# alisher-turubayev/dl-normalizing-flows

Measured on AMD Instinct MI355X. Metric: images/sec + bits/dim, RealNVP 64x64x3 training, higher is better.
Workload: dtype bf16; 1 GPU; config 1: RealNVP 64x64x3, res-blocks 4, base-dim 32, per-GPU batch 64, train step fwd+bwd+Adam; global_batch=64, image_size=64, res_blocks=4, base_dim=32, n_scales=5, parallelism=dp1, graph=True, side_stream=False

## Files before the change

### dl-normalizing-flows_amd/csrc/conv.hip

```cpp
#include <math.h>
#include <stdlib.h>

#include "common.h"
#include "conv_common.h"

#ifndef RNVP_SHARD_PX
#define RNVP_SHARD_PX 8192
#endif
extern "C" int rnvp_stat_shards(long long M) {
    long long s = M / RNVP_SHARD_PX;
    int r = 1;
    while (r < 32 && r * 2 <= s) r *= 2;
    return r;
}

namespace {

int conv_args_status(const rnvp_conv_args* a) {
    if (!a || !a->x || !a->w || !a->y) return RNVP_E_INVALID;
    if (a->variant < 0 || (a->variant > RNVP_VARIANT_DEEP && a->variant < RNVP_VARIANT_DEEP0) ||
        a->variant >= RNVP_VARIANT_DEEP0 + RNVP_DEEP_CFGS)
        return RNVP_E_INVALID;
    if (a->w_frag && !al16(a->w_frag)) return RNVP_E_INVALID;
    if (a->dtype != RNVP_F32 && a->dtype != RNVP_BF16) return RNVP_E_INVALID;
    if (a->ks != 1 && a->ks != 3) return RNVP_E_UNSUPPORTED;
    if (a->B < 0 || a->H <= 0 || a->W <= 0 || a->n <= 0 || a->cin <= 0) return RNVP_E_INVALID;
    if ((a->cs_in & 7) || (a->cs_out & 7) || a->cs_in < a->cin || a->cs_out < a->n) return RNVP_E_INVALID;
    if ((a->kp & 63) || a->kp < a->ks * a->ks * a->cs_in) return RNVP_E_INVALID;
    if (!al16(a->x) || !al16(a->w)) return RNVP_E_INVALID;
    if (a->epi_relu_bn_bwd && !a->epi_x) return RNVP_E_INVALID;
    auto tab_bad = [](const rnvp_bn_src& s) { return s.tab && (!s.sums || !al16(s.tab)); };
    if ((a->pro_bn_relu && tab_bad(a->pro)) || (a->epi_relu_bn_bwd && tab_bad(a->epi)) || (a->bp && tab_bad(a->bp_bn)))
        return RNVP_E_INVALID;
    if ((long long)a->B * a->H * a->W >= (1ll << 31)) return RNVP_E_UNSUPPORTED;
    if (a->bp) {
        if (!a->bp_x || !al16(a->bp_x) || (a->bp_out && !al16(a->bp_out))) return RNVP_E_INVALID;
        if (a->bp_bn.sums && (!a->bp_sums || a->bp_shards < 1 || a->bp_bn.count <= 0)) return RNVP_E_INVALID;
        if (!a->bp_bn.sums && (!a->bp_bn.mean || !a->bp_bn.var)) return RNVP_E_INVALID;
        if (a->pro_bn_relu) return RNVP_E_INVALID;
    }
    return RNVP_OK;
}

int bp_cfg_of(const rnvp_conv_args* a) {
    if (a->variant >= RNVP_VARIANT_DEEP0) {
        const int cfg = a->variant - RNVP_VARIANT_DEEP0;
        return (cfg == 0 || cfg == 4) ? cfg : -1;
    }
    if (a->variant != 0 && a->variant != RNVP_VARIANT_DEEP) return -1;
    const int cfg = rnvp_deep_auto_cfg(a);
    const long long M = (long long)a->B * a->H * a->W;
    if (cfg == 4 || (cfg == 0 && (a->ks == 3 || M <= 4096))) return cfg;
    return -1;
}

int dispatch_conv(const rnvp_conv_args* a, hipStream_t s, bool dry, int* fam) {
    auto ran = [&](int f, int r) {
        if (fam && r == RNVP_OK) *fam = f;
        return r;
    };
    if (a->variant >= RNVP_VARIANT_DEEP0)
        return ran(RNVP_FAMILY_DEEP, rnvp_deep_launch(a, s, a->variant - RNVP_VARIANT_DEEP0, dry));
    if (a->variant == 0 || a->variant == RNVP_VARIANT_DEEP) {
        const int cfg = rnvp_deep_auto_cfg(a);
        if (cfg >= 0) {
            const int r = rnvp_deep_launch(a, s, cfg, dry);
            if (r != RNVP_E_UNSUPPORTED) return ran(RNVP_FAMILY_DEEP, r);
        }
    }
    const bool tuned = a->variant != 1;
    if (tuned && a->dtype == RNVP_BF16 && a->ks == 1) {
        const int r = rnvp_conv_s1_launch(a, s, dry);
        if (r != RNVP_E_UNSUPPORTED) return ran(RNVP_FAMILY_S1, r);
    }
    if (tuned && rnvp_conv_band_ok(a)) {
        const int r = rnvp_conv_band2_launch(a, s, dry);
        if (r != RNVP_E_UNSUPPORTED) return ran(RNVP_FAMILY_BAND, r);
        if (dry) return ran(RNVP_FAMILY_OTHER, RNVP_OK);
        return rnvp_conv_band1_launch(a, s);
    }
    if (dry) return ran(RNVP_FAMILY_OTHER, RNVP_OK);
    {
        const int r = rnvp_conv_stream_launch(a, s);
        if (r != RNVP_E_UNSUPPORTED) return r;
    }
    if (tuned) {
        const int r = rnvp_conv_halo_launch(a, s);
        if (r != RNVP_E_UNSUPPORTED) return r;
    }
    return rnvp_conv_tiled_launch(a, s);
}

int route_conv(const rnvp_conv_args* a, hipStream_t s, bool dry, int* fam = nullptr) {
    if (a->bp) {
        const int cfg = bp_cfg_of(a);
        int r, f = RNVP_FAMILY_DEEP;
        if (cfg >= 0) {
            r = rnvp_deep_launch(a, s, cfg, dry);
        } else {
            if (a->variant != 0) return RNVP_E_UNSUPPORTED;
            f = RNVP_FAMILY_S1;
            r = rnvp_conv_s1_launch(a, s, dry);
            if (r == RNVP_E_UNSUPPORTED) {
                f = RNVP_FAMILY_BAND;
                r = rnvp_conv_band2_launch(a, s, dry);
            }
        }
        if (fam && r == RNVP_OK) *fam = f;
        return r;
    }
    return dispatch_conv(a, s, dry, fam);
}

}

extern "C" int rnvp_conv2d(const rnvp_conv_args* a, void* stream) {
    const int st = conv_args_status(a);
    if (st != RNVP_OK || a->B == 0) return st;
    return route_conv(a, (hipStream_t)stream, false);
}

extern "C" int rnvp_conv2d_family(const rnvp_conv_args* a) {
    const int st = conv_args_status(a);
    if (st != RNVP_OK) return st;
    int fam = RNVP_FAMILY_OTHER;
    const int r = route_conv(a, nullptr, true, &fam);
    return r == RNVP_OK ? fam : r;
}

extern "C" int rnvp_conv2d_check(const rnvp_conv_args* a) {
    const int st = conv_args_status(a);
    if (st != RNVP_OK || a->B == 0) return st;
    return route_conv(a, nullptr, true);
}
```

### dl-normalizing-flows_amd/csrc/conv_common.h

```cpp
#pragma once
#include <math.h>

#include "common.h"

namespace {

template <typename T> struct Mf;
template <> struct Mf<bf16_t> {
    static constexpr int CH = 8;
    __device__ static __forceinline__ void step(const u32x4& a, const u32x4& b, floatx4& c) {
        c = __builtin_amdgcn_mfma_f32_16x16x32_bf16(__builtin_bit_cast(bf16x8, a), __builtin_bit_cast(bf16x8, b), c, 0, 0, 0);
    }
};
template <> struct Mf<float> {
    static constexpr int CH = 4;
    __device__ static __forceinline__ void step(const u32x4& a, const u32x4& b, floatx4& c) {
        c = __builtin_amdgcn_mfma_f32_16x16x4f32(__uint_as_float(a.x), __uint_as_float(b.x), c, 0, 0, 0);
        c = __builtin_amdgcn_mfma_f32_16x16x4f32(__uint_as_float(a.y), __uint_as_float(b.y), c, 0, 0, 0);
        c = __builtin_amdgcn_mfma_f32_16x16x4f32(__uint_as_float(a.z), __uint_as_float(b.z), c, 0, 0, 0);
        c = __builtin_amdgcn_mfma_f32_16x16x4f32(__uint_as_float(a.w), __uint_as_float(b.w), c, 0, 0, 0);
    }
};

__device__ __forceinline__ int sw8(int row, int c) { return row * 8 + (c ^ ((row >> 1) & 7)); }
// ... 314 lines not shown
        float g[CH], x[CH], d[CH];
        unpack(vg, g, T());
        unpack(vx, x, T());
#pragma unroll
        for (int j = 0; j < CH; ++j) {
            const float* pp = p + 5 * (c0 + j);
            const float xh = (x[j] - pp[3]) * pp[4];
            d[j] = pp[0] * (g[j] - pp[1] - xh * pp[2]);
        }
        if (R) {
            float r[CH];
            unpack(vr, r, T());
#pragma unroll
            for (int j = 0; j < CH; ++j) d[j] += r[j];
        }
        if (a.accumulate) {
            float r[CH];
            unpack(vd, r, T());
#pragma unroll
            for (int j = 0; j < CH; ++j) d[j] += r[j];
        }
        *(u32x4*)(DX + o) = pack(d, T());
    };
    if (q0 < nch) apply(q0 * CH, fg, fx, fr, fd);
    for (long long q = q0 + qs; q < nch; q += qs) {
        const long long o = q * CH;
        if (!fixed) c0 = (int)(q % cpr) * CH;
        const u32x4 vg = *(const u32x4*)(G + o), vx = *(const u32x4*)(X + o);
        const u32x4 vr = R ? *(const u32x4*)(R + o) : vg;
        const u32x4 vd = a.accumulate ? *(const u32x4*)(DX + o) : vg;
        apply(o, vg, vx, vr, vd);
    }
}

template <typename T>
__device__ __forceinline__ void bn_bwd_body(const rnvp_bn_bwd_args& a, double* dsm, int blk, int nblk) {
    if (a.bn.gamma) bn_bwd_run<T, true>(a, dsm, blk, nblk);
    else bn_bwd_run<T, false>(a, dsm, blk, nblk);
}

inline bool al16(const void* p) { return (((uintptr_t)p) & 15) == 0; }

}

int rnvp_conv_tiled_launch(const rnvp_conv_args* a, hipStream_t s);

int rnvp_conv_stream_launch(const rnvp_conv_args* a, hipStream_t s);

int rnvp_conv_halo_launch(const rnvp_conv_args* a, hipStream_t s);

bool rnvp_conv_band_ok(const rnvp_conv_args* a);
int rnvp_conv_band1_launch(const rnvp_conv_args* a, hipStream_t s);

constexpr int RNVP_DEEP_CFGS = 7;
int rnvp_deep_launch(const rnvp_conv_args* a, hipStream_t s, int cfg, bool dry = false);
int rnvp_deep_auto_cfg(const rnvp_conv_args* a);

int rnvp_wgrad_tap_launch(rnvp_wgrad_group* g, hipStream_t s);
int rnvp_wgrad_tap_prepare(rnvp_wgrad_group* g);
int rnvp_wgrad_tap_multi_plan(const rnvp_wgrad_group* groups, int n_groups, int cls, rnvp_wgrad_multi_conv* convs,
                              int conv_cap, int* xcd_start, int* tasks, int task_cap, rnvp_wgrad_multi* m);
int rnvp_wgrad_tap_multi_launch(const rnvp_wgrad_multi* m, hipStream_t s);

int rnvp_conv_s1_launch(const rnvp_conv_args* a, hipStream_t s, bool dry = false);

struct rnvp_group_kargs {
    rnvp_conv_args conv[RNVP_NET_GROUP_MAX];
    int shards[RNVP_NET_GROUP_MAX], tiles[RNVP_NET_GROUP_MAX], xa[RNVP_NET_GROUP_MAX], xb[RNVP_NET_GROUP_MAX];
    int n;
};
rnvp_group_kargs group_kargs(const rnvp_net_step* steps, int n);

using GroupKernel = void (*)(const rnvp_group_kargs);
template <typename T, int CFG> int rnvp_deep_cfg_launch(const rnvp_conv_args* a, hipStream_t s, bool dry);
template <typename T, int CFG> GroupKernel rnvp_deep_cfg_group(int nc, bool fm);
int rnvp_s1_fanout_prepare(rnvp_net_step* steps, int n, int* klass, int* grid, int* lds_bytes);
int rnvp_s1_fanout_launch(const rnvp_group_kargs& g, int klass, int grid, int lds_bytes, hipStream_t s);

int rnvp_conv_band2_launch(const rnvp_conv_args* a, hipStream_t s, bool dry = false);
```

### dl-normalizing-flows_amd/csrc/conv_deep.hip

```cpp
#include "conv_deep.h"

#ifdef RNVP_DEEP_STAMPS
#include "conv_deep_launch.h"
#endif

namespace {

template <typename T>
int launch_cfg(const rnvp_conv_args* a, hipStream_t s, int cfg, bool dry) {
    switch (cfg) {
        case 0: return rnvp_deep_cfg_launch<T, 0>(a, s, dry);
        case 1: return rnvp_deep_cfg_launch<T, 1>(a, s, dry);
        case 2: return rnvp_deep_cfg_launch<T, 2>(a, s, dry);
        case 3: return rnvp_deep_cfg_launch<T, 3>(a, s, dry);
        case 4: return rnvp_deep_cfg_launch<T, 4>(a, s, dry);
        case 5: return rnvp_deep_cfg_launch<T, 5>(a, s, dry);
        case 6: return rnvp_deep_cfg_launch<T, 6>(a, s, dry);
    }
    return RNVP_E_INVALID;
}

template <typename T>
GroupKernel group_kernel_t(int cfg, int nc, bool fm) {
    switch (cfg) {
        case 0: return rnvp_deep_cfg_group<T, 0>(nc, fm);
        case 1: return rnvp_deep_cfg_group<T, 1>(nc, fm);
        case 4: return rnvp_deep_cfg_group<T, 4>(nc, fm);
        case 5: return rnvp_deep_cfg_group<T, 5>(nc, fm);
    }
    return nullptr;
}

constexpr int GROUP_FM = 1 << 11;
GroupKernel group_kernel(int dtype, int klass) {
    const int cfg = klass & 15, nc = (klass >> 4) & 127;
    const bool fm = (klass & GROUP_FM) != 0;
    return dtype == RNVP_F32 ? group_kernel_t<float>(cfg, nc, fm) : group_kernel_t<bf16_t>(cfg, nc, fm);
}

struct GroupCfg { int bn, nw, wk; };
inline GroupCfg group_cfg_shape(int cfg) {
    switch (cfg) {
        case 0: return {32, 4, 4};
        case 1: return {64, 4, 4};
        case 4: return {32, 8, 8};
        default: return {64, 8, 8};
    }
}

}

extern "C" int rnvp_net_group_prepare(rnvp_net_step* steps, int n, int* klass, int* grid, int* lds_bytes) {
    if (!steps || n <= 0 || n > RNVP_NET_GROUP_MAX || !klass || !grid || !lds_bytes) return RNVP_E_INVALID;
    const rnvp_conv_args& a0 = steps[0].conv;
    const long long M = (long long)a0.B * a0.H * a0.W;
    for (int i = 0; i < n; ++i)
        if (steps[i].conv.bp) return RNVP_E_UNSUPPORTED;
    if (M > 16384) return rnvp_s1_fanout_prepare(steps, n, klass, grid, lds_bytes);
    if (M <= 0) return RNVP_E_UNSUPPORTED;
    if (a0.dtype != RNVP_F32 && a0.dtype != RNVP_BF16) return RNVP_E_INVALID;
    const int kc = a0.dtype == RNVP_F32 ? 16 : 32;
    int cfg = -1, nc = -1;
    long long tiles = 0;
    size_t lds = 0;
    for (int i = 0; i < n; ++i) {
        rnvp_net_step& st = steps[i];
        const rnvp_conv_args& a = st.conv;
        if (st.kind != RNVP_STEP_CONV || a.ks != 1) return RNVP_E_UNSUPPORTED;
        if (a.dtype != a0.dtype || a.B != a0.B || a.H != a0.H || a.W != a0.W) return RNVP_E_UNSUPPORTED;
        if (!a.x || !a.w || !a.y || a.n <= 0 || a.cin <= 0 || (a.cs_in & 7) || (a.cs_out & 7)) return RNVP_E_INVALID;
// ... 29 lines not shown
        st.cfg = c;
        st.nc = ncv;
        st.shards = rnvp_stat_shards(M);
        st.tiles = (int)(gm * gn);
        xcd_blocks(&a, (int)gm, (int)gn, g.bn, a0.dtype == RNVP_F32 ? 4 : 2, &st.xa, &st.xb);
        tiles += st.tiles;
    }
    if (tiles <= 0 || tiles >= (1ll << 31)) return RNVP_E_INVALID;
    bool fm = a0.dtype == RNVP_BF16 && nc <= 4;
    for (int i = 0; i < n; ++i) fm = fm && steps[i].conv.w_frag != nullptr && (((uintptr_t)steps[i].conv.w_frag) & 15) == 0;
    *klass = cfg | (nc << 4) | (fm ? GROUP_FM : 0);
    *grid = (int)tiles;
    *lds_bytes = (int)lds;
    return group_kernel(a0.dtype, *klass) ? RNVP_OK : RNVP_E_UNSUPPORTED;
}

rnvp_group_kargs group_kargs(const rnvp_net_step* steps, int n) {
    rnvp_group_kargs g = {};
    for (int i = 0; i < n; ++i) {
        g.conv[i] = steps[i].conv;
        g.shards[i] = steps[i].shards;
        g.tiles[i] = steps[i].tiles;
        g.xa[i] = steps[i].xa;
        g.xb[i] = steps[i].xb;
    }
    g.n = n;
    return g;
}

extern "C" int rnvp_net_group(const rnvp_net_step* steps, int n, int dtype, int klass, int grid, int lds_bytes,
                              void* stream) {
    if (!steps || n <= 0 || n > RNVP_NET_GROUP_MAX || grid <= 0 || lds_bytes < 0 || lds_bytes > 160 * 1024)
        return RNVP_E_INVALID;
    if (dtype != RNVP_F32 && dtype != RNVP_BF16) return RNVP_E_INVALID;
    const rnvp_group_kargs g = group_kargs(steps, n);
    if (klass & (1 << 12)) {
        if (dtype != RNVP_BF16 || n < 2) return RNVP_E_INVALID;
        return rnvp_s1_fanout_launch(g, klass, grid, lds_bytes, (hipStream_t)stream);
    }
    const GroupKernel k = group_kernel(dtype, klass);
    if (!k) return RNVP_E_INVALID;
    const int nw = group_cfg_shape(klass & 15).nw;
    hipLaunchKernelGGL(k, dim3(grid), dim3(64 * nw), lds_bytes, (hipStream_t)stream, g);
    RNVP_LAUNCH_CHECK();
    return RNVP_OK;
}

int rnvp_deep_auto_cfg(const rnvp_conv_args* a) {
    const long long M = (long long)a->B * a->H * a->W;
    if (M > 16384) return -1;
    const bool dgrad = a->epi_relu_bn_bwd || (!a->pro_bn_relu && !a->out_sums);
    const int kc = a->dtype == RNVP_F32 ? 16 : 32;
    if (M <= 1024) return a->cs_in % (8 * kc) == 0 ? 4 : 0;
    if (dgrad) return 0;
    if (a->ks == 3 && a->dtype == RNVP_BF16 && M > 4096 && a->cs_in == 128) return 6;
    return a->cs_in % (8 * kc) == 0 ? 5 : 1;
}

int rnvp_deep_launch(const rnvp_conv_args* a, hipStream_t s, int cfg, bool dry) {
    if (cfg < 0 || cfg >= RNVP_DEEP_CFGS) return RNVP_E_INVALID;
    return a->dtype == RNVP_F32 ? launch_cfg<float>(a, s, cfg, dry) : launch_cfg<bf16_t>(a, s, cfg, dry);
}
```

### dl-normalizing-flows_amd/csrc/conv_deep_launch.h

```cpp
#pragma once
#include "conv_deep.h"

namespace {

template <typename T, int BN, int KSZ, bool PRO, int NW, int WK, int DK, int NC, bool FM = false, int BM = DEEP_BM,
          bool BP = false>
__global__ __launch_bounds__(64 * NW) void k_conv_deep(rnvp_conv_args a, int shards, int xa, int xb) {
    extern __shared__ __attribute__((aligned(16))) char lds[];
    deep_tile<T, BN, KSZ, PRO, NW, WK, DK, NC, FM, BM, BP>(a, shards, xa, xb, blockIdx.x, gridDim.x, lds);
}

template <int BN, int NW, int WK, int BM>
constexpr bool bp_cfg() { return BN == 32 && WK == NW && BM == DEEP_BM; }

template <typename T, int BN, int NW, int WK, int DK, int NC, int KSZ, int BM = DEEP_BM>
int launch_deep_nc(const rnvp_conv_args* a, hipStream_t s, bool dry) {
    const long long M = (long long)a->B * a->H * a->W;
    const size_t shm = deep_lds_bytes<T, BN, NW, WK, BM>(a->cs_in, a->W, a->ks, a->bp != 0);
    if (shm > 160 * 1024) return RNVP_E_UNSUPPORTED;
    const long long gm = (M + BM - 1) / BM, gn = (a->n + BN - 1) / BN;
    const unsigned grid = (unsigned)(gm * gn);
    const int sh = rnvp_stat_shards(M);
    const dim3 blk(64 * NW);
    int xa, xb;
    xcd_blocks(a, (int)gm, (int)gn, BN, sizeof(T), &xa, &xb, BM);
    if (a->bp) {
        if constexpr (bp_cfg<BN, NW, WK, BM>()) {
            if (dry) return RNVP_OK;
            if constexpr (sizeof(T) == 2 && NC <= 4) {
                if (a->w_frag) {
                    k_conv_deep<T, BN, KSZ, false, NW, WK, DK, NC, true, BM, true><<<grid, blk, shm, s>>>(*a, sh, xa, xb);
                    RNVP_LAUNCH_CHECK();
                    return RNVP_OK;
                }
            }
            k_conv_deep<T, BN, KSZ, false, NW, WK, DK, NC, false, BM, true><<<grid, blk, shm, s>>>(*a, sh, xa, xb);
            RNVP_LAUNCH_CHECK();
            return RNVP_OK;
        } else {
            return RNVP_E_UNSUPPORTED;
        }
    }
    if (dry) return RNVP_OK;
    if constexpr (sizeof(T) == 2 && NC <= 4) {
        if (a->w_frag) {
            if (a->pro_bn_relu) k_conv_deep<T, BN, KSZ, true, NW, WK, DK, NC, true, BM><<<grid, blk, shm, s>>>(*a, sh, xa, xb);
            else k_conv_deep<T, BN, KSZ, false, NW, WK, DK, NC, true, BM><<<grid, blk, shm, s>>>(*a, sh, xa, xb);
            RNVP_LAUNCH_CHECK();
            return RNVP_OK;
        }
    }
    if (a->pro_bn_relu) k_conv_deep<T, BN, KSZ, true, NW, WK, DK, NC, false, BM><<<grid, blk, shm, s>>>(*a, sh, xa, xb);
    else k_conv_deep<T, BN, KSZ, false, NW, WK, DK, NC, false, BM><<<grid, blk, shm, s>>>(*a, sh, xa, xb);
    RNVP_LAUNCH_CHECK();
// ... 49 lines not shown
        return RNVP_E_UNSUPPORTED;
    }
}

template <typename T, int BN, int NW, int WK, int DK, int NC, bool FM = false>
__global__ __launch_bounds__(64 * NW) void k_net_group(const rnvp_group_kargs g) {
    extern __shared__ __attribute__((aligned(16))) char lds[];
    int b = blockIdx.x, c = 0;
    while (c + 1 < g.n && b >= g.tiles[c]) {
        b -= g.tiles[c];
        ++c;
    }
    if (g.conv[c].pro_bn_relu)
        deep_tile<T, BN, 1, true, NW, WK, DK, NC, FM>(g.conv[c], g.shards[c], g.xa[c], g.xb[c], b, g.tiles[c], lds);
    else
        deep_tile<T, BN, 1, false, NW, WK, DK, NC, FM>(g.conv[c], g.shards[c], g.xa[c], g.xb[c], b, g.tiles[c], lds);
}

template <typename T, int BN, int NW, int WK, int DK>
GroupKernel group_kernel_nc(int nc, bool fm) {
    if constexpr (sizeof(T) == 2) {
        if (fm) {
            switch (nc) {
                case 1: return k_net_group<T, BN, NW, WK, DK, 1, true>;
                case 2: return k_net_group<T, BN, NW, WK, DK, 2, true>;
                case 4: return k_net_group<T, BN, NW, WK, DK, 4, true>;
            }
            return nullptr;
        }
    }
    if (fm) return nullptr;
    switch (nc) {
        case 1: return k_net_group<T, BN, NW, WK, DK, 1>;
        case 2: return k_net_group<T, BN, NW, WK, DK, 2>;
        case 4: return k_net_group<T, BN, NW, WK, DK, 4>;
        case 8: return k_net_group<T, BN, NW, WK, DK, 8>;
        case 16: return k_net_group<T, BN, NW, WK, DK, 16>;
    }
    return nullptr;
}

}

template <typename T, int CFG>
int rnvp_deep_cfg_launch(const rnvp_conv_args* a, hipStream_t s, bool dry) {
    static_assert(CFG >= 0 && CFG < RNVP_DEEP_CFGS, "configuration");
    if constexpr (CFG == 0) return launch_deep<T, 32, 4, 4, 8>(a, s, dry);
    if constexpr (CFG == 1) return launch_deep<T, 64, 4, 4, 6>(a, s, dry);
    if constexpr (CFG == 2) return a->ks == 1 ? launch_deep<T, 64, 4, 1, 8>(a, s, dry) : RNVP_E_UNSUPPORTED;
    if constexpr (CFG == 3) return a->ks == 1 ? launch_deep<T, 32, 4, 2, 8>(a, s, dry) : RNVP_E_UNSUPPORTED;
    if constexpr (CFG == 4) return launch_deep<T, 32, 8, 8, 8>(a, s, dry);
    if constexpr (CFG == 5) return launch_deep<T, 64, 8, 8, 6>(a, s, dry);
    if constexpr (CFG == 6) return launch_deep_tall<T, 32, 4, 4, 8>(a, s, dry);
}

template <typename T, int CFG>
GroupKernel rnvp_deep_cfg_group(int nc, bool fm) {
    static_assert(CFG == 0 || CFG == 1 || CFG == 4 || CFG == 5, "whole-tile-per-wave configurations");
    if constexpr (CFG == 0) return group_kernel_nc<T, 32, 4, 4, 8>(nc, fm);
    if constexpr (CFG == 1) return group_kernel_nc<T, 64, 4, 4, 6>(nc, fm);
    if constexpr (CFG == 4) return group_kernel_nc<T, 32, 8, 8, 8>(nc, fm);
    if constexpr (CFG == 5) return group_kernel_nc<T, 64, 8, 8, 6>(nc, fm);
}
```

### dl-normalizing-flows_amd/realnvp_hip/_lib.py

```python
import ctypes as C
import os

_HERE = os.path.dirname(os.path.abspath(__file__))
LIB_PATH = os.environ.get("RNVP_LIB_PATH") or os.path.join(_HERE, "librealnvp_hip.so")
if os.environ.get("RNVP_LIB_PATH"):
    import sys as _sys
    print("realnvp_hip: RNVP_LIB_PATH=%s replaces the in-tree library" % LIB_PATH, file=_sys.stderr)

RNVP_F32, RNVP_BF16 = 0, 1

vp = C.c_void_p
i32 = C.c_int
i64 = C.c_longlong
f32 = C.c_float
f64 = C.c_double


class BNSrc(C.Structure):
    _fields_ = [("sums", vp), ("count", f64), ("mean", vp), ("var", vp), ("gamma", vp), ("beta", vp), ("eps", f32),
                ("shards", i32), ("tab", vp)]


def bn_tab_floats(c):
    return 4 * int(c)
# ... 109 lines not shown
                ("x", vp),
                ("in_gamma", vp), ("in_beta", vp), ("in_rmean", vp), ("in_rvar", vp), ("in_nbt", vp),
                ("in_sums", vp),
                ("h0", vp), ("cs_h0", i32),
                ("st", vp), ("cs_st", i32),
                ("scale", vp), ("scale_shift", vp),
                ("u", vp), ("z", vp), ("out_sums", vp),
                ("out_rmean", vp), ("out_rvar", vp), ("out_nbt", vp),
                ("ldj_sample", vp), ("ldj_full", vp),
                ("gz", vp), ("gl_full", vp), ("gl_sample", vp), ("gx", vp),
                ("gst", vp), ("cs_gst", i32),
                ("bwd_sums", vp), ("g_scale", vp), ("g_scale_shift", vp),
                ("gh0", vp), ("cs_gh0", i32),
                ("in_bwd_sums", vp), ("g_in_gamma", vp), ("g_in_beta", vp),
                ("net_running", vp), ("n_net_running", i32), ("net_running_cmax", i32),
                ("gscale_part", vp),
                ("nclass", i32), ("cls_sums", vp), ("prior_sums", vp), ("outp_sums", vp), ("in_bwd_ext", vp),
                ("out_tab", vp), ("in_tab", vp)]


RNVP_LINK_SAME, RNVP_LINK_SQUEEZE, RNVP_LINK_UNFACTOR, RNVP_LINK_FINAL = 0, 1, 2, 3


class LinkArgs(C.Structure):
    _fields_ = [("type", i32), ("g_lp", vp), ("prior", vp), ("off", vp), ("z", vp)]


class TensorRef(C.Structure):
    _fields_ = [("p", vp), ("g", vp), ("n", i64)]


_SIGS = {
    "rnvp_version": (i32, []),
    "rnvp_struct_size": (i32, [i32]),
    "rnvp_status_string": (C.c_char_p, [i32]),
    "rnvp_marker": (i32, [i32, vp]),
    "rnvp_checkerboard_mask": (i32, [vp, i32, i32, vp]),
    "rnvp_squeeze": (i32, [vp, vp, i32, i32, i32, i32, vp]),
    "rnvp_undo_squeeze": (i32, [vp, vp, i32, i32, i32, i32, vp]),
    "rnvp_factor_out": (i32, [vp, vp, vp, i32, i32, i32, i32, vp]),
    "rnvp_restore": (i32, [vp, vp, vp, i32, i32, i32, i32, vp]),
    "rnvp_logit_fwd": (i32, [vp, vp, C.c_uint64, C.c_uint64, vp, f32, vp, vp, i32, i32, vp]),
    "rnvp_logit_inv": (i32, [vp, vp, f32, i64, vp]),
    "rnvp_u8_to_unit": (i32, [vp, vp, i64, vp]),
    "rnvp_nchw_to_nhwc": (i32, [vp, vp, i32, i32, i32, i32, i32, i32, vp]),
    "rnvp_nhwc_to_nchw": (i32, [vp, vp, i32, i32, i32, i32, i32, i32, vp]),
    "rnvp_prior_logprob": (i32, [vp, vp, vp, i32, i32, vp]),
    "rnvp_prior_logprob_bwd": (i32, [vp, vp, vp, i32, i32, vp]),
    "rnvp_bn_running_update": (i32, [vp, i32, i32, f32, vp]),
    "rnvp_stat_shards": (i32, [i64]),
    "rnvp_conv2d": (i32, [C.POINTER(ConvArgs), vp]),
    "rnvp_conv2d_check": (i32, [C.POINTER(ConvArgs)]),
    "rnvp_conv2d_family": (i32, [C.POINTER(ConvArgs)]),
    "rnvp_wgrad_slabs": (i32, [i64]),
    "rnvp_wgrad_replicas": (i32, [i32]),
    "rnvp_conv2d_wgrad_grouped": (i32, [C.POINTER(WgradGroup), vp]),
    "rnvp_wgrad_class": (i32, [C.POINTER(WgradGroup), i32]),
    "rnvp_wgrad_multi_plan": (i32, [C.POINTER(WgradGroup), i32, i32, C.POINTER(WgradMultiConv), i32, C.POINTER(i32),
                                    C.POINTER(i32), i32, C.POINTER(WgradMulti)]),
    "rnvp_conv2d_wgrad_multi": (i32, [C.POINTER(WgradMulti), vp]),
    "rnvp_wgrad_multi_struct_size": (i32, [i32]),
    "rnvp_bn_bwd_apply": (i32, [C.POINTER(BNBwdArgs), vp]),
    "rnvp_weight_norm_fwd": (i32, [vp, i32, i32, i32, i32, vp]),
    "rnvp_weight_norm_tiles": (i32, [i32, i32, i32]),
    "rnvp_weight_norm_bwd": (i32, [vp, i32, i32, vp, vp, i64, vp, i64, vp]),
    "rnvp_weight_norm_opt_blocks": (i32, [i32, i32, i32]),
    "rnvp_weight_norm_bwd_adam": (i32, [vp, i32, i32, i32, i32, C.POINTER(AdamArgs), vp, i64, vp, i64, vp]),
    "rnvp_adam_gather": (i32, [C.POINTER(AdamArgs), vp, i64, vp]),
    "rnvp_weight_norm_transpose": (i32, [vp, i32, i32, i32, vp]),
    "rnvp_zero_ranges": (i32, [vp, i32, i64, vp]),
    "rnvp_coupling_in_fwd": (i32, [C.POINTER(CouplingArgs), vp]),
    "rnvp_coupling_out_fwd": (i32, [C.POINTER(CouplingArgs), vp]),
    "rnvp_coupling_reverse": (i32, [C.POINTER(CouplingArgs), vp]),
    "rnvp_coupling_reverse_bwd": (i32, [C.POINTER(CouplingArgs), vp]),
    "rnvp_coupling_out_bwd": (i32, [C.POINTER(CouplingArgs), vp]),
    "rnvp_coupling_in_bwd": (i32, [C.POINTER(CouplingArgs), vp]),
    "rnvp_link_nclass": (i32, [i32, i32]),
    "rnvp_coupling_out_u": (i32, [C.POINTER(CouplingArgs), vp]),
    "rnvp_coupling_link_fwd": (i32, [C.POINTER(CouplingArgs), C.POINTER(CouplingArgs), C.POINTER(LinkArgs), vp]),
    "rnvp_coupling_link_bwd": (i32, [C.POINTER(CouplingArgs), C.POINTER(CouplingArgs), C.POINTER(LinkArgs), vp]),
    "rnvp_coupling_in_apply": (i32, [C.POINTER(CouplingArgs), vp]),
    "rnvp_flow_in_fwd": (i32, [vp, C.c_uint64, vp, f32, vp, vp, C.POINTER(CouplingArgs), i32, i32, i32, i32, vp]),
    "rnvp_flow_lp_finish": (i32, [vp, vp, vp, i32, vp, vp, i32, vp]),
    "rnvp_sumsq_multi": (i32, [vp, i32, vp, vp]),
    "rnvp_sumsq_bwd_multi": (i32, [vp, i32, vp, f32, vp]),
    "rnvp_adam_step": (i32, [vp, vp, vp, vp, i64, vp, f32, f32, f32, f32, f32, vp, f32, vp]),
    "rnvp_adam_update": (i32, [vp, vp, vp, vp, i64, vp, i64, f32, f32, f32, f32, f32, vp, f32, vp]),
    "rnvp_step_increment": (i32, [vp, vp]),
    "rnvp_grad_sumsq_parts": (i32, [i64]),
    "rnvp_grad_sumsq": (i32, [C.POINTER(AdamArgs), i64, vp, i32, vp]),
    "rnvp_grad_accumulate": (i32, [C.POINTER(AdamArgs), vp, i64, vp, vp, i32, vp]),
    "rnvp_step_control": (i32, [vp, vp, vp, i32, vp]),
    "rnvp_adam_range": (i32, [C.POINTER(AdamArgs), i64, vp]),
    "rnvp_step_advance": (i32, [vp, vp, vp]),
    "rnvp_ema_struct_size": (i32, []),
    "rnvp_ema_update": (i32, [vp, vp, i64, vp, vp, i64, vp, vp]),
    "rnvp_ema_swap": (i32, [vp, vp, i64, vp]),
    "rnvp_score_struct_size": (i32, []),
    "rnvp_score_in_fwd": (i32, [vp, vp, C.c_uint64, vp, f32, vp, vp, i32, i32, i32, i32, vp]),
    "rnvp_score_finish": (i32, [vp, vp, vp, vp, vp, vp, i32, i32, vp]),
    "rnvp_fill_f64": (i32, [vp, i64, f64, vp]),
    "rnvp_net_group_prepare": (i32, [vp, i32, C.POINTER(i32), C.POINTER(i32), C.POINTER(i32)]),
    "rnvp_net_group": (i32, [vp, i32, i32, i32, i32, i32, vp]),
}

EXPORTED = sorted(_SIGS)


class _Lib:
    def __init__(self, path=LIB_PATH):
        if not os.path.exists(path):
            raise RuntimeError("librealnvp_hip.so not built (%s); run __graft_entry__.build()" % path)
        self.dll = C.CDLL(path)
        for name, (res, args) in _SIGS.items():
            fn = getattr(self.dll, name)
            fn.restype = res
            fn.argtypes = args
            raw = name in ("rnvp_version", "rnvp_struct_size", "rnvp_stat_shards", "rnvp_wgrad_slabs", "rnvp_wgrad_replicas",
                           "rnvp_link_nclass", "rnvp_conv2d_check", "rnvp_conv2d_family", "rnvp_wgrad_class", "rnvp_wgrad_multi_plan", "rnvp_wgrad_multi_struct_size",
                           "rnvp_grad_sumsq_parts", "rnvp_ema_struct_size", "rnvp_score_struct_size",
                           "rnvp_weight_norm_tiles", "rnvp_weight_norm_opt_blocks",
                           "rnvp_net_group_prepare") or res is not i32
            setattr(self, name[len("rnvp_"):], fn if raw else self._wrap(name, fn))
        mirrors = (BNSrc, BNRunning, ConvArgs, WgradConv, WgradGroup, BNBwdArgs, WNDesc, AdamArgs, CouplingArgs,
                   NetStep, Range, LinkArgs, StepCtl)
        for i, m in enumerate(mirrors):
            if self.dll.rnvp_struct_size(i) != C.sizeof(m):
                raise RuntimeError("%s: struct %s is %d bytes in the library, %d in the binding (stale build?)"
                                   % (path, m.__name__, self.dll.rnvp_struct_size(i), C.sizeof(m)))
        for i, m in enumerate((WgradMultiConv, WgradMulti)):
            if self.dll.rnvp_wgrad_multi_struct_size(i) != C.sizeof(m):
                raise RuntimeError("%s: struct %s is %d bytes in the library, %d in the binding (stale build?)"
                                   % (path, m.__name__, self.dll.rnvp_wgrad_multi_struct_size(i), C.sizeof(m)))
        for m, size in ((EmaCtl, self.dll.rnvp_ema_struct_size()), (ScoreCtl, self.dll.rnvp_score_struct_size())):
            if size != C.sizeof(m):
                raise RuntimeError("%s: struct %s is %d bytes in the library, %d in the binding (stale build?)"
                                   % (path, m.__name__, size, C.sizeof(m)))

    def _wrap(self, name, fn):
        dll = self.dll

        def call(*args):
            st = fn(*args)
            if st != 0:
                msg = dll.rnvp_status_string(st)
                raise RuntimeError("%s failed: status %d (%s)" % (name, st, msg.decode() if msg else "?"))
        call.__name__ = name
        return call


_lib = None


def lib() -> _Lib:
    global _lib
    if _lib is None:
        _lib = _Lib()
    return _lib
```

### include/realnvp_hip.h

```cpp
#ifndef REALNVP_HIP_H
#define REALNVP_HIP_H

#include <stdint.h>

#ifdef __cplusplus
extern "C" {
#endif

enum { RNVP_F32 = 0, RNVP_BF16 = 1 };
enum { RNVP_OK = 0, RNVP_E_INVALID = -1, RNVP_E_UNSUPPORTED = -2 };

int rnvp_version(void);
int rnvp_struct_size(int which);
const char* rnvp_status_string(int status);
int rnvp_marker(int tag, void* stream);

int rnvp_checkerboard_mask(float* mask, int size, int config, void* stream);
int rnvp_squeeze(const float* x, float* y, int B, int C, int H, int W, void* stream);
int rnvp_undo_squeeze(const float* y, float* x, int B, int C, int H, int W, void* stream);
int rnvp_factor_out(const float* x, float* on, float* off, int B, int C, int H, int W, void* stream);
int rnvp_restore(const float* on, const float* off, float* x, int B, int C, int H, int W, void* stream);

int rnvp_logit_fwd(const float* x, const float* noise, uint64_t seed, uint64_t offset, const long long* epoch,
                   float constraint, float* y, float* logdet, int B, int n_per_sample, void* stream);
// ... 2 lines not shown
int rnvp_u8_to_unit(const uint8_t* x, float* y, long long n, void* stream);

int rnvp_nchw_to_nhwc(const float* x, void* y, int B, int C, int H, int W, int cs, int dtype, void* stream);
int rnvp_nhwc_to_nchw(const void* x, float* y, int B, int C, int H, int W, int cs, int dtype, void* stream);

int rnvp_prior_logprob(const float* z, const float* ldj, float* out, int B, int n_per_sample, void* stream);
int rnvp_prior_logprob_bwd(const float* z, const float* gout, float* gz, int B, int n_per_sample, void* stream);

typedef struct rnvp_bn_src {
    const double* sums;
    double count;
    const float* mean;
    const float* var;
    const float* gamma;
    const float* beta;
    float eps;
    int shards;
    const float* tab;
} rnvp_bn_src;
#define RNVP_BN_TAB_FLOATS(C) (4 * (C))
int rnvp_stat_shards(long long M);

typedef struct rnvp_bn_running {
    const double* sums; double count; int C; int shards;
    float* rmean; float* rvar; long long* nbt;
    float eps; float* tab;
} rnvp_bn_running;
int rnvp_bn_running_update(const rnvp_bn_running* descs_device, int n, int max_c, float momentum, void* stream);

#define RNVP_VARIANT_DEEP 2
#define RNVP_VARIANT_DEEP0 16
typedef struct rnvp_conv_args {
    int dtype;
    int B, H, W, ks;
    const void* x; int cs_in; int cin;
    const void* w; int kp;
    void* y; int cs_out; int n;
    const float* bias;
    const void* residual;
    int accumulate;
    int pro_bn_relu; rnvp_bn_src pro;
    double* out_sums;
    int epi_relu_bn_bwd; const void* epi_x; rnvp_bn_src epi; double* epi_sums;
    float* ws; long long ws_elems;
    int variant;
    const void* w_frag;
    int bp; const void* bp_x; rnvp_bn_src bp_bn; const double* bp_sums; int bp_shards;
    void* bp_out; float* bp_dgamma; float* bp_dbeta;
} rnvp_conv_args;
int rnvp_conv2d(const rnvp_conv_args* a, void* stream);
int rnvp_conv2d_check(const rnvp_conv_args* a);
enum { RNVP_FAMILY_OTHER = 0, RNVP_FAMILY_DEEP = 1, RNVP_FAMILY_S1 = 2, RNVP_FAMILY_BAND = 3 };
int rnvp_conv2d_family(const rnvp_conv_args* a);

#define RNVP_WGRAD_GROUP_MAX 24
typedef struct rnvp_wgrad_conv {
    const void* x; const void* dy;
    float* ws;
    float* wsb;
    rnvp_bn_src pro;
    int cs_in, cin, ks, cs_dy, n, kp, pro_bn_relu, nz, nrep;
    long long m_per_slab;
    int task0, tk, cls;
} rnvp_wgrad_conv;
typedef struct rnvp_wgrad_group {
    int dtype, B, H, W, n_conv;
    rnvp_wgrad_conv conv[RNVP_WGRAD_GROUP_MAX];
} rnvp_wgrad_group;
int rnvp_wgrad_slabs(long long M);
int rnvp_wgrad_replicas(int nz);
int rnvp_conv2d_wgrad_grouped(const rnvp_wgrad_group* g, void* stream);
int rnvp_wgrad_class(const rnvp_wgrad_group* g, int c);

typedef struct rnvp_wgrad_multi_conv {
    const void* x; const void* dy; float* ws; float* wsb;
    rnvp_bn_src pro;
    int cs_in, cin, cs_dy, n, kp, pro_bn_relu, nz, nrep;
    int B, H, W, cls;
    int tco, tci;
    long long m_per_slab;
} rnvp_wgrad_multi_conv;
typedef struct rnvp_wgrad_multi {
    int cls, ko, n_conv, n_task, grid, lds_bytes;
    long long xcd_cost[8];
    const rnvp_wgrad_multi_conv* convs;
    const int* xcd_start;
    const int* tasks;
} rnvp_wgrad_multi;
int rnvp_wgrad_multi_plan(const rnvp_wgrad_group* groups, int n_groups, int cls, rnvp_wgrad_multi_conv* convs,
                          int conv_cap, int* xcd_start, int* tasks, int task_cap, rnvp_wgrad_multi* m);
int rnvp_conv2d_wgrad_multi(const rnvp_wgrad_multi* m, void* stream);
int rnvp_wgrad_multi_struct_size(int which);

typedef struct rnvp_bn_bwd_args {
    int dtype; long long M; int C; int cs;
    const void* g; const void* x; rnvp_bn_src bn;
    const double* sums; int sum_shards;
    void* dx; const void* residual; int accumulate;
    float* dgamma; float* dbeta;
} rnvp_bn_bwd_args;
int rnvp_bn_bwd_apply(const rnvp_bn_bwd_args* a, void* stream);

typedef struct rnvp_wn_desc {
    const float* v; const float* g;
    void* wf; void* wd; float* norm;
    float* dw;
// ... 181 lines not shown
```

Before: 3466 images/sec.

## Add persistent tile-walking 3x3 conv kernel for narrow bf16 128-channel layers

Adds a new deep-conv config that launches persistent blocks. Each block keeps one 32-wide output-channel weight slice resident in LDS and walks a contiguous run of 64-pixel tiles. The next tile's activations (with halo) are double-buffered through registers while MFMA work proceeds on the current one. The auto-selector routes forward 3x3 bf16 convs with 128 input channels at width 8 or 16 to this kernel, with dgrad left off. This is meant to avoid reloading weights for every tile and to hide activation-load latency, at the cost of more LDS, register pressure and a fixed grid cap. It also adds a query entry point that reports which deep config would be used.

```diff
diff --git a/dl-normalizing-flows_amd/csrc/conv.hip b/dl-normalizing-flows_amd/csrc/conv.hip
--- a/dl-normalizing-flows_amd/csrc/conv.hip
+++ b/dl-normalizing-flows_amd/csrc/conv.hip
@@ -45,12 +45,12 @@
 int bp_cfg_of(const rnvp_conv_args* a) {
     if (a->variant >= RNVP_VARIANT_DEEP0) {
         const int cfg = a->variant - RNVP_VARIANT_DEEP0;
-        return (cfg == 0 || cfg == 4) ? cfg : -1;
+        return (cfg == 0 || cfg == 4 || cfg == 7) ? cfg : -1;
     }
     if (a->variant != 0 && a->variant != RNVP_VARIANT_DEEP) return -1;
     const int cfg = rnvp_deep_auto_cfg(a);
     const long long M = (long long)a->B * a->H * a->W;
-    if (cfg == 4 || (cfg == 0 && (a->ks == 3 || M <= 4096))) return cfg;
+    if (cfg == 4 || cfg == 7 || (cfg == 0 && (a->ks == 3 || M <= 4096))) return cfg;
     return -1;
 }
 
@@ -128,6 +128,17 @@
     return r == RNVP_OK ? fam : r;
 }
 
+extern "C" int rnvp_conv2d_deep_cfg(const rnvp_conv_args* a) {
+    if (conv_args_status(a) != RNVP_OK) return -1;
+    int cfg;
+    if (a->bp) cfg = bp_cfg_of(a);
+    else if (a->variant >= RNVP_VARIANT_DEEP0) cfg = a->variant - RNVP_VARIANT_DEEP0;
+    else if (a->variant == 0 || a->variant == RNVP_VARIANT_DEEP) cfg = rnvp_deep_auto_cfg(a);
+    else cfg = -1;
+    if (cfg < 0 || rnvp_deep_launch(a, nullptr, cfg, true) != RNVP_OK) return -1;
+    return cfg;
+}
+
 extern "C" int rnvp_conv2d_check(const rnvp_conv_args* a) {
     const int st = conv_args_status(a);
     if (st != RNVP_OK || a->B == 0) return st;
diff --git a/dl-normalizing-flows_amd/csrc/conv_common.h b/dl-normalizing-flows_amd/csrc/conv_common.h
--- a/dl-normalizing-flows_amd/csrc/conv_common.h
+++ b/dl-normalizing-flows_amd/csrc/conv_common.h
@@ -390,7 +390,7 @@
 bool rnvp_conv_band_ok(const rnvp_conv_args* a);
 int rnvp_conv_band1_launch(const rnvp_conv_args* a, hipStream_t s);
 
-constexpr int RNVP_DEEP_CFGS = 7;
+constexpr int RNVP_DEEP_CFGS = 8;
 int rnvp_deep_launch(const rnvp_conv_args* a, hipStream_t s, int cfg, bool dry = false);
 int rnvp_deep_auto_cfg(const rnvp_conv_args* a);
 
diff --git a/dl-normalizing-flows_amd/csrc/conv_deep.hip b/dl-normalizing-flows_amd/csrc/conv_deep.hip
--- a/dl-normalizing-flows_amd/csrc/conv_deep.hip
+++ b/dl-normalizing-flows_amd/csrc/conv_deep.hip
@@ -16,6 +16,9 @@
         case 4: return rnvp_deep_cfg_launch<T, 4>(a, s, dry);
         case 5: return rnvp_deep_cfg_launch<T, 5>(a, s, dry);
         case 6: return rnvp_deep_cfg_launch<T, 6>(a, s, dry);
+        case 7:
+            if constexpr (sizeof(T) == 2) return rnvp_deep_cfg_launch<T, 7>(a, s, dry);
+            else return RNVP_E_UNSUPPORTED;
     }
     return RNVP_E_INVALID;
 }
@@ -151,6 +154,10 @@
     const bool dgrad = a->epi_relu_bn_bwd || (!a->pro_bn_relu && !a->out_sums);
     const int kc = a->dtype == RNVP_F32 ? 16 : 32;
     if (M <= 1024) return a->cs_in % (8 * kc) == 0 ? 4 : 0;
+    constexpr bool WALK_FWD = true, WALK_DGRAD = false;
+    if (a->ks == 3 && a->dtype == RNVP_BF16 && M > 4096 && a->cs_in == 128 && (a->W == 8 || a->W == 16) && a->n >= 16 &&
+        (dgrad ? WALK_DGRAD : WALK_FWD))
+        return 7;
     if (dgrad) return 0;
     if (a->ks == 3 && a->dtype == RNVP_BF16 && M > 4096 && a->cs_in == 128) return 6;
     return a->cs_in % (8 * kc) == 0 ? 5 : 1;
diff --git a/dl-normalizing-flows_amd/csrc/conv_deep_launch.h b/dl-normalizing-flows_amd/csrc/conv_deep_launch.h
--- a/dl-normalizing-flows_amd/csrc/conv_deep_launch.h
+++ b/dl-normalizing-flows_amd/csrc/conv_deep_launch.h
@@ -1,5 +1,6 @@
 #pragma once
 #include "conv_deep.h"
+#include "conv_deep_walk.h"
 
 namespace {
 
@@ -155,6 +156,7 @@
     if constexpr (CFG == 4) return launch_deep<T, 32, 8, 8, 8>(a, s, dry);
     if constexpr (CFG == 5) return launch_deep<T, 64, 8, 8, 6>(a, s, dry);
     if constexpr (CFG == 6) return launch_deep_tall<T, 32, 4, 4, 8>(a, s, dry);
+    if constexpr (CFG == 7) return launch_deep_walk<T>(a, s, dry);
 }
 
 template <typename T, int CFG>
diff --git a/dl-normalizing-flows_amd/csrc/conv_deep_walk.h b/dl-normalizing-flows_amd/csrc/conv_deep_walk.h
--- /dev/null
+++ b/dl-normalizing-flows_amd/csrc/conv_deep_walk.h
@@ -0,0 +1,373 @@
+#pragma once
+#include <type_traits>
+
+#include "conv_deep.h"
+
+namespace {
+
+constexpr int WALK_BM = 64;
+constexpr int WALK_BN = 32;
+constexpr int WALK_CS = 128;
+constexpr int WALK_NT = 256;
+constexpr int WALK_MAXW = 16;
+#ifndef WALK_PF
+#define WALK_PF 4
+#endif
+
+template <int N, int I = 0, typename F>
+__device__ __forceinline__ void walk_static_for(F&& f) {
+    if constexpr (I < N) {
+        f(std::integral_constant<int, I>{});
+        walk_static_for<N, I + 1>(f);
+    }
+}
+
+constexpr int walk_kpl() { return lds_mfma_pitch(9 * WALK_CS, 8); }
+
+inline size_t walk_lds_bytes(int W) {
+    const int R = WALK_BM + 2 * (W + 1), pitch = lds_mfma_pitch(WALK_CS, 8);
+    return 4 * (5 * (size_t)WALK_BN) + 8 * (2 * 2 * (size_t)WALK_BN) + 4 * 5 * (size_t)WALK_CS +
+           2 * ((size_t)pitch + (size_t)WALK_BN * walk_kpl() + 2 * (size_t)R * pitch);
+}
+
+__host__ __device__ inline void walk_run(int nt, int npg, int i, int* t0, int* t1) {
+    const int base = nt / npg, rem = nt - base * npg;
+    *t0 = i * base + (i < rem ? i : rem);
+    *t1 = *t0 + base + (i < rem ? 1 : 0);
+}
+
+template <bool PRO, bool BP, bool FM, bool WREG>
+__global__ __launch_bounds__(WALK_NT) void k_conv_walk(rnvp_conv_args a, int shards, int npg) {
+    using T = bf16_t;
+    constexpr int NT = WALK_NT, CH = 8, KS = 32, BM = WALK_BM, BN = WALK_BN, cs = WALK_CS;
+    constexpr int NSTEP = 9 * cs / KS;
+    constexpr int KPL = walk_kpl();
+    constexpr int pitch = lds_mfma_pitch(cs, CH);
+    constexpr int TMW = 2;
+    constexpr int CPR = cs / CH, RSTEP = NT / CPR;
+    constexpr int SB = (BM + 2 * (WALK_MAXW + 1) + RSTEP - 1) / RSTEP;
+    constexpr int WB = BN * (9 * cs / CH) / NT;
+    static_assert(WB * NT == BN * 9 * cs / CH, "weight chunks");
+    static_assert(!(BP && PRO), "BatchNorm-backward prologue: data gradients only");
+    extern __shared__ __attribute__((aligned(16))) char lds[];
+    const int tid = threadIdx.x, lane = tid & 63, g = lane >> 4, li = lane & 15;
+    const int wid = __builtin_amdgcn_readfirstlane(tid >> 6);
+    const int pg = wid & 1, hf = wid >> 1;
+    const int M = a.B * a.H * a.W, W = a.W, H = a.H;
+    const int N = a.n, cso = a.cs_out;
+    const int ntile = (M + BM - 1) / BM;
+    const int nb = gridDim.x, b = blockIdx.x;
+    const int q8 = nb / 8, r8 = nb % 8, xcd = b % 8;
+    const int t = (xcd < r8 ? xcd * (q8 + 1) : r8 * (q8 + 1) + (xcd - r8) * q8) + b / 8;
+    const int slice = t / npg, n0 = slice * BN;
+    int t0, t1;
+    walk_run(ntile, npg, t - slice * npg, &t0, &t1);
+    if (t0 >= t1) return;
+    const bool epi_bn = a.epi_relu_bn_bwd != 0;
+    const int hal = W + 1, R = BM + 2 * hal;
+
+    float* etab = (float*)lds;
+    float* btab = etab + 4 * BN;
+    double* sred = (double*)(btab + BN);
+    float* bnp = (float*)(sred + 2 * BN * 2);
+    T* zrow = (T*)(bnp + 5 * cs);
+    T* Wl = zrow + pitch;
+    T* act0 = Wl + BN * KPL;
+
+    const T* __restrict__ X = (const T*)a.x;
+    const T* __restrict__ XT = (const T*)a.bp_x;
+    T* __restrict__ BPO = (T*)a.bp_out;
+    const bool bp_store = BP && BPO != nullptr && slice == 0;
+    const int cfix = tid % CPR, rbase = tid / CPR;
+    u32x4 sv[SB];
+    u32x4 sx[BP ? SB : 1];
+    auto stage_load = [&](int tile) {
+        const int m0 = tile * BM;
+#pragma unroll
+        for (int u = 0; u < SB; ++u) {
+            if (u * RSTEP >= R) break;
+            const int r = rbase + u * RSTEP;
+            const int p = m0 - hal + r;
+            const bool ok = (r < R) & (p >= 0) & (p < M);
+            const long long o = ok ? (long long)p * cs + cfix * CH : 0;
+            sv[u] = *(const u32x4*)(X + o);
+            if constexpr (BP) sx[u] = *(const u32x4*)(XT + o);
+        }
+    };
+    float scv[CH], shv[CH];
+    auto stage_store = [&](int tile, T* act) {
+        const int m0 = tile * BM;
+        float bco[BP ? CH : 1], bk1[BP ? CH : 1], bk2[BP ? CH : 1], bmo[BP ? CH : 1], bro[BP ? CH : 1];
+        if constexpr (BP) {
+#pragma unroll
+            for (int e = 0; e < CH; ++e) {
+                bco[e] = bnp[cfix * CH + e];
+                bk1[e] = bnp[cs + cfix * CH + e];
+                bk2[e] = bnp[2 * cs + cfix * CH + e];
+                bmo[e] = bnp[3 * cs + cfix * CH + e];
+                bro[e] = bnp[4 * cs + cfix * CH + e];
+            }
+        }
+#pragma unroll
+        for (int u = 0; u < SB; ++u) {
+            if (u * RSTEP >= R) break;
+            const int r = rbase + u * RSTEP;
+            if (r >= R) continue;
+            const int p = m0 - hal + r;
+            u32x4 w = sv[u];
+            if (PRO) w = bn_relu_bf16x8(w, scv, shv);
+            if constexpr (BP) {
+                float gv[CH], xv[CH], d[CH];
+                unpack(w, gv, T());
+                unpack(sx[u], xv, T());
+#pragma unroll
+                for (int e = 0; e < CH; ++e) {
+                    const float xh = (xv[e] - bmo[e]) * bro[e];
+                    d[e] = bco[e] * fmaf(-xh, bk2[e], gv[e] - bk1[e]);
+                }
+                w = pack(d, T());
+                if (bp_store && r >= hal && r < hal + BM && p < M) *(u32x4*)(BPO + (long long)p * cs + cfix * CH) = w;
+            }
+            const uint32_t keep = (p >= 0 && p < M) ? ~0u : 0u;
+            *(u32x4*)(act + r * pitch + cfix * CH) = w & u32x4{keep, keep, keep, keep};
+        }
+    };
+
+    DEEP_STAMP(0);
+    BnTab<1> ptab, etb;
+    if (PRO) tab_issue<1, NT>(a.pro, a.cin, 0, cs, ptab);
+    BnTab<1> btb, gtb;
+    rnvp_bn_src gsrc = {};
+    if constexpr (BP) {
+        gsrc.sums = a.bp_sums;
+        gsrc.count = a.bp_bn.count;
+        gsrc.shards = a.bp_shards;
+        rnvp_bn_src bsrc = a.bp_bn;
+        if (bsrc.tab) bsrc.tab += 2 * BN_TAB_DIV;
+        tab_issue<1, NT>(bsrc, a.cin, 0, cs, btb);
+        tab_issue<1, NT>(gsrc, a.cin, 0, cs, gtb);
+    }
+    if (epi_bn) tab_issue<1, NT>(a.epi, N, n0, BN, etb);
+    const float bval = (tid < BN && a.bias && n0 + tid < N) ? a.bias[n0 + tid] : 0.f;
+    stage_load(t0);
+    const T* __restrict__ Wg = (const T*)(FM ? a.w_frag : a.w);
+    u32x4 wv[WB];
+    int wdst[WB];
+#pragma unroll
+    for (int u = 0; u < WB; ++u) {
+        const int q = u * NT + tid;
+        if constexpr (FM) {
+            const int blk = q >> 6, e = q & 63, rb = blk / NSTEP, kb = blk - rb * NSTEP;
+            const int nbk = (n0 >> 4) + rb, nbl = (N + 15) >> 4;
+            wv[u] = *(const u32x4*)(Wg + ((long long)(nbk < nbl ? nbk : 0) * (a.kp >> 5) + kb) * 512 + e * CH);
+            wdst[u] = (rb * 16 + (e & 15)) * KPL + kb * KS + (e >> 4) * CH;
+        } else {
+            constexpr int wcpr = 9 * cs / CH;
+            const int r = q / wcpr, c = q - r * wcpr;
+            wv[u] = *(const u32x4*)(Wg + (long long)(n0 + r < N ? n0 + r : 0) * a.kp + c * CH);
+            wdst[u] = r * KPL + c * CH;
+        }
+    }
+    if (PRO) tab_finish<1, NT>(a.pro, a.cin, 0, cs, ptab, bnp, bnp + cs, nullptr, nullptr);
+    if constexpr (BP) {
+        const int c = tid;
+        if (c < cs) {
+            float coef = 0.f, k1 = 0.f, k2 = 0.f, mo = 0.f, ro = 1.f;
+            if (c < a.cin) {
+                if (a.bp_bn.tab) {
+                    const unsigned long long u = (unsigned long long)__double_as_longlong(btb.a1[0]);
+                    mo = __uint_as_float((unsigned)u);
+                    ro = __uint_as_float((unsigned)(u >> 32));
+                    coef = btb.gam[0] * ro;
+                } else {
+                    double mean, var;
+                    if (a.bp_bn.sums) {
+                        const double s1 = btb.a1[0] + (a.bp_bn.shards > 1 ? btb.b1[0] : 0.0);
+                        const double s2 = btb.a2[0] + (a.bp_bn.shards > 1 ? btb.b2[0] : 0.0);
+                        mean = s1 / a.bp_bn.count;
+                        var = s2 / a.bp_bn.count - mean * mean;
+                        if (var < 0) var = 0;
+                    } else {
+                        mean = btb.a1[0];
+                        var = btb.a2[0];
+                    }
+                    ro = (float)(1.0 / sqrt(var + (double)a.bp_bn.eps));
+                    mo = (float)mean;
+                    coef = btb.gam[0] * ro;
+                }
+                const double g1 = gtb.a1[0] + (a.bp_shards > 1 ? gtb.b1[0] : 0.0);
+                const double g2 = gtb.a2[0] + (a.bp_shards > 1 ? gtb.b2[0] : 0.0);
+                if (a.bp_bn.sums) {
+                    k1 = (float)(g1 / a.bp_bn.count);
+                    k2 = (float)(g2 / a.bp_bn.count);
+                }
+                if (b == 0) {
+                    if (a.bp_dbeta) a.bp_dbeta[c] = (float)g1;
+                    if (a.bp_dgamma) a.bp_dgamma[c] = (float)g2;
+                }
+            }
+            bnp[c] = coef;
+            bnp[cs + c] = k1;
+            bnp[2 * cs + c] = k2;
+            bnp[3 * cs + c] = mo;
+            bnp[4 * cs + c] = ro;
+        }
+    }
+    if (epi_bn) tab_finish<1, NT>(a.epi, N, n0, BN, etb, etab, etab + BN, etab + 2 * BN, etab + 3 * BN);
+    if (tid < BN) btab[tid] = bval;
+    for (int c = tid * CH; c < pitch; c += NT * CH) *(u32x4*)(zrow + c) = u32x4{0u, 0u, 0u, 0u};
+#pragma unroll
+    for (int u = 0; u < WB; ++u) *(u32x4*)(Wl + wdst[u]) = wv[u];
+    __syncthreads();
+    DEEP_STAMP(1);
+    if (PRO) {
+#pragma unroll
+        for (int e = 0; e < CH; ++e) {
+            scv[e] = bnp[cfix * CH + e];
+            shv[e] = bnp[cs + cfix * CH + e];
+        }
+    }
+    stage_store(t0, act0);
+    const T* wl = Wl + (hf * 16 + li) * KPL + g * CH;
+    u32x4 wr[WREG ? NSTEP : 1];
+    if constexpr (WREG) {
+#pragma unroll
+        for (int st = 0; st < NSTEP; ++st) wr[st] = *(const u32x4*)(wl + st * KS);
+    }
+    __syncthreads();
+    DEEP_STAMP(2);
+
+    const float rW = 1.0f / (float)W, rH = 1.0f / (float)H;
+    const int col = hf * 16 + 4 * g;
+    const int n = n0 + col;
+    double s1[4], s2[4];
+#pragma unroll
+    for (int r = 0; r < 4; ++r) s1[r] = s2[r] = 0.0;
+
+    for (int tile = t0; tile < t1; ++tile) {
+        const int cur = (tile - t0) & 1;
+        const T* act = act0 + cur * R * pitch;
+        const bool more = tile + 1 < t1;
+        if (more) stage_load(tile + 1);
+        const int m0 = tile * BM;
+        EpiPre pre[TMW];
+#pragma unroll
+        for (int i = 0; i < TMW; ++i) {
+            const int m = m0 + (pg * TMW + i) * 16 + li;
+            epi_prefetch<T>(a, (long long)m * cso + n, m < M && n < cso, pre[i]);
+        }
+        int rowoff[TMW];
+        unsigned tvm[TMW];
+#pragma unroll
+        for (int i = 0; i < TMW; ++i) {
+            const int lp = (pg * TMW + i) * 16 + li, m = m0 + lp;
+            rowoff[i] = (lp + hal) * pitch + g * CH;
+            const int mm = m < M ? m : 0;
+            const int row = fdiv_small(mm, rW);
+            const int x = mm - row * W, y = row - fdiv_small(row, rH) * H;
+            tvm[i] = tap_mask<3>(x, y, W, H, m < M);
+        }
+        floatx4 acc[TMW][4];
+#pragma unroll
+        for (int i = 0; i < TMW; ++i)
+#pragma unroll
+            for (int c = 0; c < 4; ++c) acc[i][c] = floatx4{0.f, 0.f, 0.f, 0.f};
+        constexpr int PF = WALK_PF, RG = PF + 1;
+        u32x4 wf[WREG ? 1 : RG], av[RG][TMW];
+        auto frag = [&](auto STC) {
+            constexpr int st = decltype(STC)::value;
+            constexpr int tp = st / 4, ch = st % 4, buf = st % RG;
+            if constexpr (!WREG) wf[buf] = *(const u32x4*)(wl + st * KS);
+            const int toff = ((tp / 3 - 1) * W + (tp % 3 - 1)) * pitch + ch * KS;
+#pragma unroll
+            for (int i = 0; i < TMW; ++i)
+                av[buf][i] = *(const u32x4*)(((tvm[i] >> tp) & 1u) ? act + rowoff[i] + toff : zrow + ch * KS);
+        };
+        walk_static_for<PF>([&](auto STC) { frag(STC); });
+        walk_static_for<NSTEP>([&](auto STC) {
+            constexpr int st = decltype(STC)::value;
+            if constexpr (st + PF < NSTEP) frag(std::integral_constant<int, st + PF>{});
+            __builtin_amdgcn_sched_barrier(0);
+#pragma unroll
+            for (int i = 0; i < TMW; ++i) {
+                if constexpr (WREG) Mf<T>::step(wr[st], av[st % RG][i], acc[i][st % 4]);
+                else Mf<T>::step(wf[st % RG], av[st % RG][i], acc[i][st % 4]);
+            }
+            __builtin_amdgcn_sched_barrier(0);
+        });
+        if (tile == t0) DEEP_STAMP(3);
+#pragma unroll
+        for (int i = 0; i < TMW; ++i) {
+            const int m = m0 + (pg * TMW + i) * 16 + li;
+            if (m >= M || n >= cso) continue;
+            floatx4 v = acc[i][0];
+            v += acc[i][1];
+            v += acc[i][2];
+            v += acc[i][3];
+            epi4p<T>(a, (long long)m * cso + n, v, btab + col, epi_bn, etab + col, BN, s1, s2, N - n, pre[i]);
+        }
+        if (tile == t0) DEEP_STAMP(6);
+        if (more) stage_store(tile + 1, act0 + (cur ^ 1) * R * pitch);
+        __syncthreads();
+        if (tile == t0) DEEP_STAMP(7);
+    }
+    DEEP_STAMP(4);
+
+    const bool want_sums = a.out_sums || (epi_bn && a.epi_sums);
+    if (want_sums) {
+#pragma unroll
+        for (int r = 0; r < 4; ++r) {
+            const double u1 = row_sum16(s1[r]), u2 = row_sum16(s2[r]);
+            if (li == 0) {
+                sred[(pg * BN + col + r) * 2] = u1;
+                sred[(pg * BN + col + r) * 2 + 1] = u2;
+            }
+        }
+        __syncthreads();
+        double* sums = (epi_bn ? a.epi_sums : a.out_sums) + (long long)(b % shards) * 2 * N;
+        if (tid < BN && n0 + tid < N) {
+            atomicAdd(&sums[n0 + tid], sred[tid * 2] + sred[(BN + tid) * 2]);
+            atomicAdd(&sums[N + n0 + tid], sred[tid * 2 + 1] + sred[(BN + tid) * 2 + 1]);
+        }
+    }
+    DEEP_STAMP(5);
+}
+
+template <typename T>
+int launch_deep_walk(const rnvp_conv_args* a, hipStream_t s, bool dry) {
+    if constexpr (sizeof(T) != 2) {
+        return RNVP_E_UNSUPPORTED;
+    } else {
+        const long long M = (long long)a->B * a->H * a->W;
+        if (a->ks != 3 || a->cs_in != WALK_CS || (a->W != 8 && a->W != 16)) return RNVP_E_UNSUPPORTED;
+        if (M > 65536 || a->n < WALK_BN / 2) return RNVP_E_UNSUPPORTED;
+        if (a->pro_bn_relu && a->pro.sums && a->pro.shards > 2) return RNVP_E_UNSUPPORTED;
+        if (a->epi_relu_bn_bwd && a->epi.sums && a->epi.shards > 2) return RNVP_E_UNSUPPORTED;
+        if (a->bp && (a->pro_bn_relu || (a->bp_bn.sums && a->bp_bn.shards > 2) || a->bp_shards > 2)) return RNVP_E_UNSUPPORTED;
+        const size_t shm = walk_lds_bytes(a->W);
+        if (shm > 160 * 1024) return RNVP_E_UNSUPPORTED;
+        if (dry) return RNVP_OK;
+        const int ntile = (int)((M + WALK_BM - 1) / WALK_BM), gn = (a->n + WALK_BN - 1) / WALK_BN;
+        const int cap = gn < 256 ? 256 / gn : 1;
+        const int npg = ntile < cap ? ntile : cap;
+        const unsigned grid = (unsigned)(gn * npg);
+        const int sh = rnvp_stat_shards(M);
+        const dim3 blk(WALK_NT);
+        const bool fm = a->w_frag != nullptr;
+        constexpr bool WR = false;
+        if (a->bp) {
+            if (fm) k_conv_walk<false, true, true, WR><<<grid, blk, shm, s>>>(*a, sh, npg);
+            else k_conv_walk<false, true, false, WR><<<grid, blk, shm, s>>>(*a, sh, npg);
+        } else if (a->pro_bn_relu) {
+            if (fm) k_conv_walk<true, false, true, WR><<<grid, blk, shm, s>>>(*a, sh, npg);
+            else k_conv_walk<true, false, false, WR><<<grid, blk, shm, s>>>(*a, sh, npg);
+        } else {
+            if (fm) k_conv_walk<false, false, true, WR><<<grid, blk, shm, s>>>(*a, sh, npg);
+            else k_conv_walk<false, false, false, WR><<<grid, blk, shm, s>>>(*a, sh, npg);
+        }
+        RNVP_LAUNCH_CHECK();
+        return RNVP_OK;
+    }
+}
+
+}
diff --git a/dl-normalizing-flows_amd/realnvp_hip/_lib.py b/dl-normalizing-flows_amd/realnvp_hip/_lib.py
--- a/dl-normalizing-flows_amd/realnvp_hip/_lib.py
+++ b/dl-normalizing-flows_amd/realnvp_hip/_lib.py
@@ -185,6 +185,7 @@
     "rnvp_conv2d": (i32, [C.POINTER(ConvArgs), vp]),
     "rnvp_conv2d_check": (i32, [C.POINTER(ConvArgs)]),
     "rnvp_conv2d_family": (i32, [C.POINTER(ConvArgs)]),
+    "rnvp_conv2d_deep_cfg": (i32, [C.POINTER(ConvArgs)]),
     "rnvp_wgrad_slabs": (i32, [i64]),
     "rnvp_wgrad_replicas": (i32, [i32]),
     "rnvp_conv2d_wgrad_grouped": (i32, [C.POINTER(WgradGroup), vp]),
@@ -250,7 +251,7 @@
             fn.restype = res
             fn.argtypes = args
             raw = name in ("rnvp_version", "rnvp_struct_size", "rnvp_stat_shards", "rnvp_wgrad_slabs", "rnvp_wgrad_replicas",
-                           "rnvp_link_nclass", "rnvp_conv2d_check", "rnvp_conv2d_family", "rnvp_wgrad_class", "rnvp_wgrad_multi_plan", "rnvp_wgrad_multi_struct_size",
+                           "rnvp_link_nclass", "rnvp_conv2d_check", "rnvp_conv2d_family", "rnvp_conv2d_deep_cfg", "rnvp_wgrad_class", "rnvp_wgrad_multi_plan", "rnvp_wgrad_multi_struct_size",
                            "rnvp_grad_sumsq_parts", "rnvp_ema_struct_size", "rnvp_score_struct_size",
                            "rnvp_weight_norm_tiles", "rnvp_weight_norm_opt_blocks",
                            "rnvp_net_group_prepare") or res is not i32
diff --git a/include/realnvp_hip.h b/include/realnvp_hip.h
--- a/include/realnvp_hip.h
+++ b/include/realnvp_hip.h
@@ -78,6 +78,7 @@
 int rnvp_conv2d_check(const rnvp_conv_args* a);
 enum { RNVP_FAMILY_OTHER = 0, RNVP_FAMILY_DEEP = 1, RNVP_FAMILY_S1 = 2, RNVP_FAMILY_BAND = 3 };
 int rnvp_conv2d_family(const rnvp_conv_args* a);
+int rnvp_conv2d_deep_cfg(const rnvp_conv_args* a);
 
 #define RNVP_WGRAD_GROUP_MAX 24
 typedef struct rnvp_wgrad_conv {
```

After: 3487 images/sec, median of 6. About the same (+0.6%).
